# Atomu2014/deep-ctr

Measured on AMD Instinct MI355X. Metric: examples/sec, higher is better.
Workload: dtype bf16; 1 GPU; FNN L3 train step: 16 fields, 937670 one-hot dims, k=10, hidden 300/100 tanh, batch 4096 per GPU, Zipf(1.1) ids; per_gpu_batch=4096, global_batch=4096, parallelism=single

## Files before the change

### deep-ctr_amd/_capi.py

```python
import ctypes as C
import os

_HERE = os.path.dirname(os.path.abspath(__file__))
LIB_PATH = os.environ.get("FNN_HIP_LIB") or os.path.join(_HERE, "libfnn_hip.so")

FNN_OK = 0
FNN_ERR_ARG, FNN_ERR_HIP, FNN_ERR_STATE, FNN_ERR_RANGE, FNN_ERR_NOMEM = -1, -2, -3, -4, -5
FNN_PREC_F32, FNN_PREC_BF16, FNN_PREC_BF16X3 = 0, 1, 2
PRECISIONS = {'f32': FNN_PREC_F32, 'bf16': FNN_PREC_BF16, 'bf16x3': FNN_PREC_BF16X3}
FNN_ACT_TANH, FNN_ACT_SIGMOID, FNN_ACT_LINEAR = 0, 1, 2
FNN_MEM_HOST, FNN_MEM_DEVICE = 0, 1
FNN_MODE_FM, FNN_MODE_BAG = 0, 1
FNN_DP_SPARSE_LOCAL, FNN_DP_SPARSE_EXCHANGE = 0, 1
FNN_DP_PAYLOAD_SLABS, FNN_DP_PAYLOAD_BUCKET = 0, 1
FNN_DP_COLLECTIVE_CALLBACK, FNN_DP_COLLECTIVE_P2P = 0, 1
ALLREDUCE_FN = C.CFUNCTYPE(C.c_int, C.c_void_p, C.c_void_p, C.c_int64, C.c_void_p)
ALLGATHER_FN = C.CFUNCTYPE(C.c_int, C.c_void_p, C.c_void_p, C.c_void_p, C.c_int64, C.c_void_p)


class fnn_cfg(C.Structure):
    _fields_ = [("n_fields", C.c_int32), ("k", C.c_int32), ("hidden1", C.c_int32),
                ("hidden2", C.c_int32), ("max_batch", C.c_int32), ("precision", C.c_int32),
                ("act", C.c_int32), ("reg_all", C.c_int32), ("lr", C.c_float),
                ("lambda1", C.c_float), ("lambda_fm", C.c_float), ("device", C.c_int32),
                ("stream", C.c_void_p), ("mode", C.c_int32), ("h0", C.c_int32)]


_vp, _i, _i64, _f = C.c_void_p, C.c_int, C.c_int64, C.c_float

SIGNATURES = {
    "fnn_version": (C.c_char_p, []),
    "fnn_cfg_size": (C.c_uint64, []),
    "fnn_last_error": (C.c_char_p, [_vp]),
    "fnn_create": (_i, [C.POINTER(fnn_cfg), C.POINTER(_vp)]),
    "fnn_destroy": (_i, [_vp]),
    "fnn_set_hparams": (_i, [_vp, _f, _f, _f]),
    "fnn_stream": (_vp, [_vp]),
    "fnn_sync": (_i, [_vp]),
    "fnn_set_table": (_i, [_vp, _vp, _i64, _vp, _f, _i]),
    "fnn_get_table": (_i, [_vp, _vp, _i]),
    "fnn_get_rows": (_i, [_vp, _vp, _i64, _vp, _i]),
    "fnn_set_dense": (_i, [_vp, _i, _vp, _vp, _i]),
    "fnn_get_dense": (_i, [_vp, _i, _vp, _vp, _i]),
    "fnn_set_bag_bias": (_i, [_vp, _vp, _i]),
    "fnn_get_bag_bias": (_i, [_vp, _vp, _i]),
    "fnn_gather": (_i, [_vp, _vp, _i, _vp, _i]),
    "fnn_train_step": (_i, [_vp, _vp, _vp, _i, _vp, _vp, _i, _vp, _vp, _i, C.POINTER(_f)]),
    "fnn_set_shadowed": (_i, [_vp, _vp, _i, _i]),
# ... 147 lines not shown
```

### deep-ctr_amd/csrc/fm_api.hip

```cpp
#include <hip/hip_runtime.h>

#include <cmath>
#include <cstring>
#include <string>
#include <vector>

#include "../../include/fm_hip.h"
#include "../../include/fnn_hip.h"
#include "fnn_step_kernels.hip.h"
#include "metrics.hip.h"
#include "optim.hip.h"

using namespace fnn;

namespace {

thread_local std::string g_fm_err;
inline int rup(int x, int m) { return (x + m - 1) / m * m; }

struct FmArgs {
    const int32_t* ids; const float* y; int B, F, K; const float* table16; int64_t n_rows; const float* b;
    float scale, dscale; int train; float* gxp; int K1p; float* p_out; float* loss_t; float* gb_part; int* err;
    bool wt;
    int* stamp; int step;
// ... 312 lines not shown
}

}

struct fm_handle {
    std::string err; int dev = 0; hipStream_t st = nullptr; bool own_stream = false;
    int F = 0, K = 0, Bmax = 0, K1p = 0;
    bool wide = false;
    int rw = SLOT;
    int* noshare = nullptr;
    float* table16 = nullptr; int64_t n_rows = 0; float* b = nullptr; double scale = 1.0;
    float *gxp = nullptr, *loss_t = nullptr, *gb_part = nullptr, *loss_dev = nullptr; int* err_flag = nullptr;
    int4* rec = nullptr; double* part = nullptr; int4* owners = nullptr; int* owner_cnt = nullptr; void* skeys = nullptr;
    double* cpow1 = nullptr; bool key64 = true;
    int opt = FM_OPT_SGD; float beta1 = 0.9f, beta2 = 0.999f, eps = 1e-8f; int64_t t = 0; bool dense_g = false;
    int scat_slot = 0;
    int sort_merge4 = 0;
    float *s0 = nullptr, *s1 = nullptr, *sb = nullptr, *G = nullptr; int* stamp = nullptr;
};

#define MHK(h, expr) do { hipError_t e_ = (expr); if (e_ != hipSuccess) { (h)->err = std::string(#expr) + ": " + hipGetErrorString(e_); return FNN_ERR_HIP; } } while (0)
#define MFAIL(h, code, msg) do { (h)->err = (msg); return (code); } while (0)

namespace {

int fold_scale(fm_handle* h)
{
    if (h->scale == 1.0 || !h->table16) return FNN_OK;
    const size_t n = (size_t)h->n_rows * h->rw;
    hipLaunchKernelGGL(k_fm_rescale, dim3((unsigned)((n + 255) / 256)), dim3(256), 0, h->st, h->table16, n, (float)h->scale);
    MHK(h, hipGetLastError());
// ... 127 lines not shown
    }
    {
        SortArgs so{ids, B, F, h->n_rows, h->rec, h->owner_cnt, 4 * F, h->skeys};
        so.merge4 = h->sort_merge4;
        SortArgs sb = so; sb.nblk = 16 * F;
        if (h->key64) {
            hipLaunchKernelGGL((k_sortA<unsigned long long>), dim3(4 * F), dim3(256), sortA_lds_bytes<unsigned long long>(so.merge4), h->st, so);
            launch_fwd<unsigned long long>(h, &sb, a, Ba / 16);
        } else {
            hipLaunchKernelGGL((k_sortA<unsigned>), dim3(4 * F), dim3(256), sortA_lds_bytes<unsigned>(so.merge4), h->st, so);
            launch_fwd<unsigned>(h, &sb, a, Ba / 16);
        }
    }
    if (opt) {
        ScatArgs sa{h->rec, SORT_N, F, h->K, h->gxp, h->K1p, h->cpow1, -1.0, h->G, h->part, h->owner_cnt, h->owners, SLOT};
        const int nsc1 = scat1_blocks(sa, h->scat_slot);
        hipLaunchKernelGGL(k_scat1, dim3(nsc1), dim3(256), 0, h->st, sa);
        hipLaunchKernelGGL(k_fm_scat2_tail, dim3(1 + 256), dim3(256), 0, h->st, sa, h->b, h->gb_part, Ba / 16, lr, lambda, h->loss_t, Ba,
                           reduce_mean ? 1.0f / (float)B : 1.0f, h->loss_dev, FmBiasOpt{h->opt, h->sb, lr_step, h->beta1, h->beta2, h->eps});
        launch_opt_pass(h, lambda, lr_step);
        MHK(h, hipGetLastError());
        return FNN_OK;
    }
    h->scale *= 1.0 - (double)lr * (double)lambda;
    ScatArgs sa{h->rec, SORT_N, F, h->K, h->gxp, h->K1p, h->cpow1, (double)lr / h->scale, h->table16, h->part, h->owner_cnt,
                h->owners, SLOT};
    const int nsc1 = scat1_blocks(sa, h->scat_slot);
    hipLaunchKernelGGL(k_scat1, dim3(nsc1), dim3(256), 0, h->st, sa);
    hipLaunchKernelGGL(k_fm_scat2_tail, dim3(1 + 256), dim3(256), 0, h->st, sa, h->b, h->gb_part, Ba / 16, lr, lambda, h->loss_t, Ba,
                       reduce_mean ? 1.0f / (float)B : 1.0f, h->loss_dev, FmBiasOpt{FM_OPT_SGD, nullptr, 0.f, 0.f, 0.f, 0.f});
    MHK(h, hipGetLastError());
    if (h->scale < 5.96e-8 || h->scale > 1.0) return fold_scale(h);
    return FNN_OK;
}

}

extern "C" {

const char* fm_last_error(const fm_handle* h) { return h ? h->err.c_str() : g_fm_err.c_str(); }

int fm_create(int n_fields, int k, int max_batch, int device, void* stream, fm_handle** out)
// ... 16 lines not shown
    const size_t Ba = rup(h->Bmax, 16);
    FK(al((void**)&h->gxp, Ba * h->K1p * 4)); FK(al((void**)&h->loss_t, Ba * 4)); FK(al((void**)&h->gb_part, (Ba / 8) * 4));
    FK(al((void**)&h->loss_dev, 4)); FK(al((void**)&h->b, 4)); FK(al((void**)&h->err_flag, 4)); FK(al((void**)&h->sb, 8));
    const size_t part_rows = h->wide ? (size_t)h->F * (SORT_N / WCH) * 2 : (size_t)h->F * (SORT_N / 16) * 2;
    FK(al((void**)&h->rec, (size_t)h->F * SORT_N * sizeof(int4))); FK(al((void**)&h->part, part_rows * h->rw * 8));
    FK(al((void**)&h->owners, (size_t)h->F * (SORT_N / 16) * sizeof(int4))); FK(al((void**)&h->owner_cnt, 4));
    FK(al(&h->skeys, (size_t)h->F * SORT_N * 8));
    {
        std::vector<double> ones(SORT_N + 1, 1.0);
        FK(hipMalloc((void**)&h->cpow1, ones.size() * 8));
        FK(hipMemcpy(h->cpow1, ones.data(), ones.size() * 8, hipMemcpyHostToDevice));
    }
    FK(hipStreamSynchronize(h->st));
#undef FK
    h->dense_g = getenv("FM_OPT_DENSE_G") && atoi(getenv("FM_OPT_DENSE_G")) == 1;
    h->scat_slot = scat1_form_env();
    h->sort_merge4 = sort_merge4_env(0);
    *out = h;
    return FNN_OK;
}

int fm_destroy(fm_handle* h)
{
    if (!h) return FNN_ERR_ARG;
    hipSetDevice(h->dev);
    if (h->st) hipStreamSynchronize(h->st);
    void* ptrs[] = {h->table16, h->b, h->gxp, h->loss_t, h->gb_part, h->loss_dev, h->err_flag, h->rec, h->part, h->owners, h->owner_cnt,
                    h->skeys, h->cpow1, h->s0, h->s1, h->sb, h->G, h->stamp, h->noshare};
    for (void* p : ptrs) if (p) hipFree(p);
    if (h->own_stream && h->st) hipStreamDestroy(h->st);
    delete h;
// ... 175 lines not shown
```

### deep-ctr_amd/csrc/fnn_api.hip

```cpp
#include <hip/hip_runtime.h>
#include <rccl/rccl.h>
#include <dlfcn.h>

#include <algorithm>

#include <cmath>
#include <cstdio>
#include <cstdlib>
#include <cstring>
#include <map>
#include <mutex>
#include <string>
#include <vector>

#include "../../include/fnn_hip.h"
#include "fnn_step_kernels.hip.h"
#include "metrics.hip.h"

using namespace fnn;

namespace {

thread_local std::string g_create_err;

// ... 5 lines not shown
}

struct fnn_handle {
    fnn_cfg cfg{};
    std::string err;
    int dev = 0;
    hipStream_t st = nullptr;
    bool own_stream = false;
    int F = 0, K = 0, H1 = 0, H2 = 0, xdim = 0, K1p = 0, H1p = 0, H2p = 0;
    int Bmax = 0, ldT = 0, N2max = 0;
    size_t n1 = 0, n2 = 0, nw12 = 0, nw = 0;
    int splitk = 4;
    int scat2_wgs = 256;
    int sort_merge4 = 1;
    int wgrad_lds = 0;
    int scat_slot = 0;
    bool bf16 = false;
    bool split = false;
    int step1_waves = 8;
    int wt_stores = 47;
    bool bag = false; int rw = SLOT; size_t nbag = 0, off_bag = 0;
    bool wide = false;
    float* bb0 = nullptr; void* dlxT = nullptr; void* onesT = nullptr; float* gx_raw = nullptr;
    bool fused = true;
    int role_off = 0;
    float* table16 = nullptr; int32_t* field_of_row = nullptr; int64_t n_rows = 0; float w0 = 0.f;
    float* master = nullptr; float* bucket = nullptr; float* slab = nullptr;
    void *w1 = nullptr, *w1t = nullptr, *w2 = nullptr, *w2t = nullptr;
    bool dense_set[3] = {false, false, false};
    void *xp = nullptr, *xpT = nullptr, *d1 = nullptr, *d1T = nullptr, *d2 = nullptr, *dl2 = nullptr,
         *dl2T = nullptr, *dl1 = nullptr, *dl1T = nullptr;
// ... 209 lines not shown
}

template <typename T>
void launch_step2(fnn_handle* h, bool dense, bool sparse, const float* gxp_src = nullptr)
{
    const int Ba = h->pend_Ba, nxt = h->cur ^ 1;
    const bool have_next = sparse && h->pend_have_next && !(h->role_off & 1);
    if (h->role_off & 2) dense = false;
    if (h->role_off & 4) sparse = false;
    ScatArgs sa = make_scat_args(h, h->slot[h->cur], SORT_N);
    if (gxp_src) sa.gxp = gxp_src;
    ProfScope ps(h, dense && sparse ? "step2" : (dense ? "step2_dense" : "step2_sparse"), h->st);
    const WgradArgs wa = make_wgrad_args<T>(h, Ba);
    const int nwx = dense ? wgrad_blocks(wa) : 0;
    const int nsc = !sparse ? 0 : (h->bag ? (int)(((size_t)h->F * (SORT_N / WCH) * (h->rw / 4) + 255) / 256)
                                          : scat1_blocks(sa, h->scat_slot));
    SortArgs so{h->next_ids, h->next_B, h->F, h->n_rows, h->slot[nxt].rec, h->slot[nxt].owner_cnt,
                have_next ? 4 * h->F : 0, h->skeys, nullptr, nullptr, 0, h->sort_merge4};
    const dim3 grid(so.nblk + nwx * h->splitk + nsc);
    if (grid.x == 0) return;
    const bool wl = nwx > 0 && h->wgrad_lds && sizeof(T) == 2;
    const size_t lds = std::max(h->key64 ? sortA_lds_bytes<unsigned long long>(so.merge4) : sortA_lds_bytes<unsigned>(so.merge4),
                                wl ? WGRAD_LDS_BYTES : (size_t)0);
#define STEP2(KT, M4, WF) hipLaunchKernelGGL((k_step2<T, KT, M4, WF>), grid, dim3(256), lds, h->st, so, wa, nwx, h->splitk, sa)
#define STEP2_KEYS(WF) do { if (h->key64) { if (so.merge4) STEP2(unsigned long long, true, WF); else STEP2(unsigned long long, false, WF); } \
                            else { if (so.merge4) STEP2(unsigned, true, WF); else STEP2(unsigned, false, WF); } } while (0)
    if constexpr (sizeof(T) == 2) {
        if (wl) { STEP2_KEYS(WGRAD_LDS); return; }
    }
    STEP2_KEYS(WGRAD_DIRECT);
#undef STEP2_KEYS
// ... 289 lines not shown
        sa.gxf = h->rw;
        {
            ProfScope ps(h, "scatter", h->st);
            const size_t nthr = (size_t)F * (N2 / WCH) * (h->rw / 4);
            hipLaunchKernelGGL(k_scatdw1, dim3((unsigned)((nthr + 255) / 256)), dim3(256), 0, h->st, sa);
        }
        {
            ProfScope ps(h, "finalize", h->st);
            hipLaunchKernelGGL(k_scatdw2, dim3(256), dim3(256), 0, h->st, sa);
        }
        HIPCHK(h, hipGetLastError());
        return FNN_OK;
    }
    {
        ProfScope ps(h, "scatter", h->st);
        const int nblk = scat1_blocks(sa, h->scat_slot);
        hipLaunchKernelGGL(k_scat1, dim3(nblk), dim3(256), 0, h->st, sa);
    }
    {
        ProfScope ps(h, "finalize", h->st);
        hipLaunchKernelGGL(k_scat2, dim3(64), dim3(256), 0, h->st, sa);
    }
    HIPCHK(h, hipGetLastError());
    return FNN_OK;
}

int ensure_global_ws(fnn_handle* h, int B_g)
{
    int N2 = sort_n2(B_g);
    if (N2 <= h->gN2 && h->cpow_cap >= B_g + 1) return FNN_OK;
    HIPCHK(h, hipStreamSynchronize(h->st));
// ... 34 lines not shown
            std::string err;
            if (group_global(h->st, ids_g, B_g, F, h->n_rows, N2, sl.rec, sl.owner_cnt, &h->gws, &h->gws_bytes, err) != 0)
                FAIL(h, FNN_ERR_HIP, err);
        } else {
            const int kpt = N2 <= 4096 ? 4 : (N2 == 8192 ? 8 : 16);
            const dim3 blk(N2 / kpt);
            if (kpt == 4) hipLaunchKernelGGL(k_sort<4>, dim3(F), blk, (size_t)N2 * 8, h->st, ids_g, B_g, F, h->n_rows, N2, sl.rec, sl.owner_cnt, nullptr, 0, h->err_flag);
            else if (kpt == 8) hipLaunchKernelGGL(k_sort<8>, dim3(F), blk, (size_t)N2 * 8, h->st, ids_g, B_g, F, h->n_rows, N2, sl.rec, sl.owner_cnt, nullptr, 0, h->err_flag);
            else hipLaunchKernelGGL(k_sort<16>, dim3(F), blk, (size_t)N2 * 8, h->st, ids_g, B_g, F, h->n_rows, N2, sl.rec, sl.owner_cnt, nullptr, 0, h->err_flag);
        }
    }
    {
        ProfScope ps(h, "scatter_global", h->st);
        ScatArgs sa = make_scat_args(h, sl, N2);
        sa.gxp = gxp_g;
        const int nblk = scat1_blocks(sa, h->scat_slot);
        hipLaunchKernelGGL(k_scat1, dim3(nblk), dim3(256), 0, h->st, sa);
        hipLaunchKernelGGL(k_scat2, dim3(N2 > 4096 ? 256 : 64), dim3(256), 0, h->st, sa);
    }
    HIPCHK(h, hipGetLastError());
    h->next_ids = nullptr; h->next_B = 0;
    h->scatter_pending = false;
    return FNN_OK;
}

struct RcclApi {
    void* lib = nullptr;
    decltype(&ncclGetUniqueId) GetUniqueId = nullptr;
    decltype(&ncclCommInitRank) CommInitRank = nullptr;
    decltype(&ncclAllReduce) AllReduce = nullptr;
    decltype(&ncclAllGather) AllGather = nullptr;
// ... 81 lines not shown
    if (!h->table16) FAIL(h, FNN_ERR_STATE, "fnn_set_table has not been called");
    if (!(h->dense_set[0] && h->dense_set[1] && h->dense_set[2]))
        FAIL(h, FNN_ERR_STATE, "fnn_set_dense has not been called for all three layers");
    return FNN_OK;
}

}

extern "C" {

const char* fnn_version(void) { return "fnn_hip 0.2 (gfx950)"; }

uint64_t fnn_cfg_size(void) { return (uint64_t)sizeof(fnn_cfg); }

const char* fnn_last_error(const fnn_handle* h) { return h ? h->err.c_str() : g_create_err.c_str(); }

int fnn_create(const fnn_cfg* cfg, fnn_handle** out)
{
    if (!cfg || !out) { g_create_err = "null argument"; return FNN_ERR_ARG; }
    *out = nullptr;
    if (cfg->n_fields < 2 || cfg->n_fields > 64) { g_create_err = "n_fields must be in [2, 64]"; return FNN_ERR_ARG; }
    if (cfg->mode != FNN_MODE_FM && cfg->mode != FNN_MODE_BAG) { g_create_err = "bad mode"; return FNN_ERR_ARG; }
    if (cfg->mode == FNN_MODE_BAG && (cfg->h0 < 192 || cfg->h0 > 316 || cfg->h0 % 4 != 0)) {
        g_create_err = "FNN_MODE_BAG: h0 must be a multiple of 4 in [192, 316] (the strip kernel is built for bag rows of 256 or 320 padded floats; the reference uses 200 and 300, python/SNN_RBM.py:25,53)"; return FNN_ERR_ARG; }
    if (cfg->mode == FNN_MODE_FM && (cfg->k < 1 || cfg->k > 128 || cfg->k == 16)) {
        g_create_err = "k = rank+1 must be in [1, 15] (two pad slots of the 16-float row carry w_0 and the bias) or in [17, 128] (wide rows of rup(k, 4) floats); k = 16 is not supported"; return FNN_ERR_ARG; }
    if (cfg->mode == FNN_MODE_FM && cfg->k >= 17 && cfg->n_fields * rup(cfg->k, 4) > WIDE_XW_MAX) {
        g_create_err = "k >= 17: n_fields * rup(k, 4) must be <= 4096 (the layer-one width of the wide-row path)"; return FNN_ERR_ARG; }
    if (cfg->hidden1 < 1 || cfg->hidden1 > 4095 || cfg->hidden2 < 1 || cfg->hidden2 > 255) { g_create_err = "hidden1 must be in [1, 4095], hidden2 in [1, 255]"; return FNN_ERR_ARG; }
    if (cfg->max_batch < 1 || cfg->max_batch > 16384) { g_create_err = "max_batch must be in [1, 16384] (per-field LDS sort)"; return FNN_ERR_ARG; }
// ... 20 lines not shown
    h->xdim = 1 + h->F * h->K;
    h->K1p = rup(h->F * SLOT, 64); h->H1p = rup(h->H1 + 1, 64); h->H2p = rup(h->H2 + 1, 64);
    h->bag = cfg->mode == FNN_MODE_BAG;
    if (const char* e = getenv("FNN_WT_STORES")) h->wt_stores = atoi(e);
    if (const char* e = getenv("FNN_STEP1_WAVES")) h->step1_waves = atoi(e) == 4 ? 4 : 8;
    if (h->bag) { h->rw = cfg->h0; h->K = cfg->h0; h->xdim = cfg->h0; h->K1p = rup(cfg->h0 + 1, 64); }
    h->wide = !h->bag && h->K >= 17;
    if (h->wide) { h->rw = rup(h->K, 4); h->K1p = rup(h->F * h->rw + 2, 64); }
    h->Bmax = cfg->max_batch; h->ldT = rup(h->Bmax, 256);
    h->N2max = SORT_N; while (h->N2max < h->Bmax) h->N2max <<= 1;
    h->n1 = (size_t)h->K1p * h->H1p; h->n2 = (size_t)h->H1p * h->H2p;
    h->nw12 = h->n1 + h->n2; h->nw = h->nw12 + h->H2p;
    h->bf16 = cfg->precision == FNN_PREC_BF16; h->split = cfg->precision == FNN_PREC_BF16X3;
    if (const char* ev = getenv("FNN_NO_FUSE")) h->fused = !(ev[0] == '1');
    if (const char* ev = getenv("FNN_ROLE_OFF")) h->role_off = atoi(ev);
    h->scat_slot = scat1_form_env();
    h->sort_merge4 = sort_merge4_env(h->bag ? 0 : 1);
    const bool steps3 = h->fused && mlp_shape_ok(h) && !h->bag && !h->scat_slot && !h->split && h->Bmax <= SORT_N;
    if (steps3) h->splitk = 8;
    const bool lds_dflt = steps3 && h->bf16 && h->ldT / 4 / Traits<bf16_t>::KS >= WGRAD_LDS_S;
    h->wgrad_lds = wgrad_form == WGRAD_LDS || (wgrad_form == -1 && lds_dflt) ? 1 : 0;
    if (wgrad_form == -1 && lds_dflt) h->splitk = 4;
    if (const char* ev = getenv("FNN_SPLITK")) { const int v = atoi(ev); if (v == 2 || v == 4 || v == 8 || v == 16) h->splitk = v; }
    if (const char* ev = getenv("FNN_SCAT2_WGS")) { const int v = atoi(ev); if (v >= 16 && v <= 1024) h->scat2_wgs = v; }
    const size_t ts = tsize(h), Ba = h->ldT;
    CK(alloc_dev(h, &h->master, h->nw));
    h->off_bag = h->nw12 + (size_t)h->H2p * 64;
    h->nbag = h->bag ? (size_t)h->K1p : 0;
    CK(alloc_dev(h, &h->bucket, h->nw + h->nbag));
    h->nslab = h->off_bag + h->nbag * 64;
    CK(alloc_dev(h, &h->slab, (size_t)h->splitk * h->nslab));
    CK(alloc_dev(h, (char**)&h->w1, h->n1 * ts));   CK(alloc_dev(h, (char**)&h->w1t, h->n1 * ts));
    CK(alloc_dev(h, (char**)&h->w2, h->n2 * ts));   CK(alloc_dev(h, (char**)&h->w2t, h->n2 * ts));
// ... 763 lines not shown
```

### deep-ctr_amd/csrc/fnn_kernels.hip.h

```cpp
#pragma once
#include <hip/hip_runtime.h>
#include <stdint.h>
#include <stdlib.h>
#include <string.h>
#include <type_traits>

namespace fnn {

typedef __bf16 bf16_t;
typedef __bf16 bf16x8 __attribute__((ext_vector_type(8)));
typedef __bf16 bf16x4 __attribute__((ext_vector_type(4)));
typedef float f32x4 __attribute__((ext_vector_type(4)));

constexpr int SLOT = 16;
constexpr int ACT_TANH = 0, ACT_SIGMOID = 1, ACT_LINEAR = 2;
constexpr double FIX_SCALE = 17592186044416.0;

__host__ __device__ inline unsigned bs_pack(const float v) {
    const bf16_t h = (bf16_t)v;
    const bf16_t l = (bf16_t)(v - (float)h);
    return (unsigned)__builtin_bit_cast(unsigned short, h) | (unsigned)__builtin_bit_cast(unsigned short, l) << 16;
}
__host__ __device__ inline float bs_unpack(const unsigned u) {
    return __builtin_bit_cast(float, u << 16) + __builtin_bit_cast(float, u & 0xffff0000u);
// ... 1619 lines not shown
            const int s = lo;
            lo = pos + 1; hi = N2;
            while (lo < hi) { const int mid = (lo + hi) >> 1; if (s_key[mid] < hi_key) lo = mid + 1; else hi = mid; }
            r = make_int4((int)(kk >> 32), (int)(kk & 0xffffffffu), s, lo);
        }
        rec[(size_t)f * N2 + pos] = r;
    }
}

struct ScatArgs {
    const int4* rec; int N2, F, K; const float* gxp; int K1p; const double* cpow; double lr;
    float* table16; double* part; int* owner_cnt; int4* owners;
    int rw;
    const int* tag_shared; int stamp;
    int gxf;
    int slot_form;
};
__device__ __forceinline__ void atomic_add4(float* p, float a, float b, float c, float d) {
    atomicAdd(p, a); atomicAdd(p + 1, b); atomicAdd(p + 2, c); atomicAdd(p + 3, d);
}
__device__ __forceinline__ void scat1_body(const ScatArgs& sa, const int blk)
{
    const int4* __restrict__ rec = sa.rec; const int N2 = sa.N2, F = sa.F, K = sa.K, K1p = sa.K1p;
    const float* __restrict__ gxp = sa.gxp; const double* __restrict__ cpow = sa.cpow; const double lr = sa.lr;
    float* __restrict__ table16 = sa.table16; double* __restrict__ part = sa.part;
    int* __restrict__ owner_cnt = sa.owner_cnt; int4* __restrict__ owners = sa.owners;
    const int l = threadIdx.x & 15;
    const int G = (blk * 256 + threadIdx.x) >> 4;
    const int NQ = N2 >> 4;
    if (G >= F * NQ) return;
    const int f = G / NQ, q = G % NQ, base = q * 16;
    const int4 mine = rec[(size_t)f * N2 + base + l];
// ... 89 lines not shown
                    if (lim < 3) o.z = wold[j].z;
                    o.w = wold[j].w;
                }
                *reinterpret_cast<float4*>(sa.table16 + (size_t)r[j].x * SLOT + 4 * q) = o;
            } else {
                const int which = (s < base) ? 0 : 1;
                double* pp = sa.part + (((size_t)f * NQ + qc) * 2 + which) * SLOT + 4 * q;
                pp[0] = a0; pp[1] = a1; pp[2] = a2; pp[3] = a3;
                if (which == 1 && q == 0) sa.owners[atomicAdd(sa.owner_cnt, 1)] = make_int4(f, s, e, r[j].x);
            }
            a0 = a1 = a2 = a3 = 0;
        }
    }
}

static __global__ __launch_bounds__(256) void k_scat1(const ScatArgs sa)
{
    if (sa.slot_form) scat1_body(sa, blockIdx.x);
    else scat1q_body(sa, blockIdx.x);
}

inline int scat1_blocks(ScatArgs& sa, const int slot_form)
{
    const bool vec_ok = ((uintptr_t)sa.gxp | (uintptr_t)sa.table16) % 16 == 0 && sa.K1p % 4 == 0;
    sa.slot_form = (slot_form || !vec_ok) ? 1 : 0;
    const size_t nthr = sa.slot_form ? (size_t)sa.F * sa.N2 : (size_t)sa.F * (sa.N2 / 16) * ((sa.K + 3) / 4);
    return (int)((nthr + 255) / 256);
}
inline int scat1_form_env()
{
    const char* e = getenv("FNN_SCAT1_FORM");
    return e && !strcmp(e, "slot") ? 1 : 0;
}

__device__ __forceinline__ void scat2_body(const ScatArgs& sa, const int blk, const int nblk, double (*s_sum)[16])
{
    const int4* __restrict__ owners = sa.owners; const int N2 = sa.N2, K = sa.K;
    const double* __restrict__ part = sa.part; const double* __restrict__ cpow = sa.cpow; const double lr = sa.lr;
    float* __restrict__ table16 = sa.table16;
    const int n = *sa.owner_cnt;
    const int l = threadIdx.x & 15, grp = threadIdx.x >> 4;
    const int NQ = N2 >> 4;
    for (int o = blk; o < n; o += nblk) {
        const int4 ow = owners[o];
        const int q0 = ow.y >> 4, q1 = (ow.z - 1) >> 4;
        double sum = 0.0;
        float* p = table16 + (size_t)ow.w * SLOT + l;
// ... 311 lines not shown
```

### deep-ctr_amd/csrc/fnn_step_kernels.hip.h

```cpp
#pragma once
#include "fnn_kernels.hip.h"

namespace fnn {

template <typename KT> struct KeyTraits;
template <> struct KeyTraits<unsigned> { static constexpr int SH = 12; };
template <> struct KeyTraits<unsigned long long> { static constexpr int SH = 32; };

struct SortArgs {
    const int32_t* ids; int B, F; int64_t n_rows; int4* rec; int* owner_cnt; int nblk; void* skeys;
    int* tag_first; int* tag_shared; int stamp;
    int merge4;
};

constexpr int SORT_N = 4096;

template <typename KT> __host__ __device__ constexpr size_t sort_lds_bytes() { return (size_t)SORT_N * sizeof(KT); }
template <typename KT> inline size_t sortA_lds_bytes(const int merge4) { return merge4 ? (size_t)1024 * sizeof(KT) : 0; }
inline int sort_merge4_env(const int dflt)
{
    const char* e = getenv("FNN_SORT_RUNS");
    const int v = e ? atoi(e) : 0;
    return v == 16 ? 0 : (v == 4 ? 1 : dflt);
}
// ... 191 lines not shown
static __global__ __launch_bounds__(256) void k_step2(const SortArgs so, const WgradArgs wa, const int nwx,
                                               const int splitk, const ScatArgs sa)
{
    extern __shared__ __align__(16) unsigned char smem[];
    const int b = blockIdx.x, nw = nwx * splitk;
    if (b < so.nblk) sortA_form<KT, M4>(so, b, smem);
    else if (b < so.nblk + nw) {
        int w = b - so.nblk;
        if (((b ^ w) & 7) == 0) {
            const int cls = w & 7, k = w >> 3, qd = nw >> 3, rm = nw & 7;
            w = (cls < rm ? cls * (qd + 1) : rm * (qd + 1) + (cls - rm) * qd) + k;
        }
        wgrad_body<T, WF>(wa, w % nwx, w / nwx, smem);
    }
    else if (sa.rw != SLOT) scatw1_body(sa, b - so.nblk - nw);
    else if (sa.slot_form) scat1_body(sa, b - so.nblk - nw);
    else scat1q_body(sa, b - so.nblk - nw);
}

struct TailArgs {
    const float* slab; int splitk; size_t nw_all, nw12, nslab; float* master; float lambda1; int reg_all;
    const float* loss_t; int Ba; float* bucket; float* loss_sum; float lr; int K1p, H1p, H2p;
    void *w1, *w1t, *w2, *w2t; int nblk_red;
    float* bb0; size_t nbag, off_bag;
};

template <typename T, bool UPDATE, typename KT, bool M4>
static __global__ __launch_bounds__(256) void k_step3(const SortArgs so, const TailArgs ta, const ScatArgs sa)
{
    extern __shared__ __align__(16) unsigned char smem[];
    __shared__ double s_sum[16][16];
// ... 148 lines not shown
```

### deep-ctr_amd/csrc/ipnn_api.hip

```cpp
#include <hip/hip_runtime.h>

#include <algorithm>
#include <cmath>
#include <cstring>
#include <map>
#include <string>
#include <vector>

#include "../../include/fnn_hip.h"
#include "../../include/ipnn_hip.h"
#include "fnn_step_kernels.hip.h"
#include "metrics.hip.h"
#include "optim.hip.h"

using namespace fnn;

namespace {

thread_local std::string g_ip_err;
inline int rup(int x, int m) { return (x + m - 1) / m * m; }

constexpr int A_TANH = IPNN_ACT_TANH, A_SIG = IPNN_ACT_SIGMOID, A_RELU = IPNN_ACT_RELU;

__device__ inline float ip_act(float z, int act) {
// ... 1337 lines not shown
    bool upd_side = false, tab_pending = false, upd_pending = false;
    float* emb = nullptr;
    float *dz0 = nullptr, *gxp = nullptr, *gb_part = nullptr, *loss_t = nullptr, *loss_dev = nullptr, *slab = nullptr;
    int* ref0 = nullptr; int* err_flag = nullptr;
    int4* rec = nullptr; double* part = nullptr; int4* owners = nullptr; int* owner_cnt = nullptr; void* skeys = nullptr;
    double* cpow1 = nullptr; bool key64 = true;
    size_t slab_stride = 0;
    bool prof = false;
    long long* stamps = nullptr;
    bool group_wgrad = true;
    bool strip_attr = false;
    int mask_side = 0;
    int group_xcd = 1;
    int strip_rot = 1, fwd_skip = 0;
    int wide_nf = 2, wide_nw = 8;
    int scat_slot = 0;
    int sort_merge4 = 1;
    bool wt = true;
    int tail_fuse = 1;
    int tail_nf = 1;
    int tail_nw = 16;
    int ipf_nt = 1024;
    int strip_warm = 1;
    bool strip = true;
    int duo = 1, duo_min = DUO_MIN_BLOCKS;
    unsigned long long* duo_xch = nullptr; int* duo_flags = nullptr; int duo_epoch = 0; size_t duo_xch_wg = 0; int n_cu = 256;
    bool stamp_tail = false;
    int tail_split = 1;
    bool duo_failed = false;
    bool gemm_lds = false;
    std::map<std::string, std::vector<std::pair<hipEvent_t, hipEvent_t>>> prof_ev;
// ... 395 lines not shown
            }
            hipLaunchKernelGGL(k_ip_b_update, dim3(1), dim3(256), 0, ss, h->b, h->gb_part, ngb, h->adam ? (int)h->cfg.optimizer : 0, h->bmv,
                               lr_step, h->cfg.adam_beta1, h->cfg.adam_beta2, h->cfg.adam_eps, h->err_flag);
        }
        if (h->wide) {
            IpProf ps(h, "scatter", ss);
            ScatArgs sa{h->rec, SORT_N, F, h->K, h->gxp, h->Dp[0], h->cpow1, h->adam ? -1.0 : (double)h->cfg.lr,
                        h->adam ? h->tG : h->table16, h->part, h->owner_cnt, h->owners, h->rw, h->noshare, 1, h->rw};
            const int nthr = F * (SORT_N / WCH) * (h->rw / 4);
            hipLaunchKernelGGL(k_ip_scatw1, dim3((nthr + 255) / 256), dim3(256), 0, ss, sa);
            hipLaunchKernelGGL(k_ip_scatw2, dim3(256), dim3(256), 0, ss, sa);
        } else {
            IpProf ps(h, "scatter", ss);
            ScatArgs sa{h->rec, SORT_N, F, h->K, h->gxp, h->Dp[0], h->cpow1, h->adam ? -1.0 : (double)h->cfg.lr,
                        h->adam ? h->tG : h->table16, h->part, h->owner_cnt, h->owners, SLOT};
            const int nsc1 = scat1_blocks(sa, h->scat_slot);
            hipLaunchKernelGGL(k_scat1, dim3(nsc1), dim3(256), 0, ss, sa);
            hipLaunchKernelGGL(k_scat2, dim3(256), dim3(256), 0, ss, sa);
        }
        if (h->adam) {
            IpProf ps(h, "adam_table", ss);
            const size_t n = (size_t)h->n_rows * h->rw;
            hipLaunchKernelGGL(k_adam_table, dim3((unsigned)((n / 4 + 255) / 256)), dim3(256), 0, ss, h->table16, h->tm, h->tv, h->tG, n,
                               lr_step, h->cfg.adam_beta1, h->cfg.adam_beta2, h->cfg.adam_eps, (int)h->cfg.optimizer);
        }
        if (h->st2) IHK(h, hipEventRecord(h->st2 && h->upd_side ? h->ev_tab : h->ev_join, h->st2));
    }
    {
        IpProf ps(h, "wgrad");
        if (h->group_wgrad && L + 1 <= GEMM_GROUP_MAX) {
            GemmGroupArgs g{};
// ... 80 lines not shown
    h->wide = h->K > SLOT; h->rw = h->wide ? rup(h->K, 4) : SLOT;
    h->P = cfg->pairs ? h->F * (h->F - 1) / 2 : 0; h->CB = h->F * h->rw + h->P; h->bf16 = cfg->precision == FNN_PREC_BF16;
    h->Bmax = cfg->max_batch; h->ldT = rup(h->Bmax, 256);
    if (const char* e = getenv("IPNN_GEMM_LDS")) h->gemm_lds = atoi(e) != 0;
    if (const char* e = getenv("IPNN_STRIP")) h->strip = atoi(e) != 0;
    if (const char* e = getenv("IPNN_STRIP_DUO")) h->duo = atoi(e);
    if (const char* e = getenv("IPNN_DUO_MIN")) h->duo_min = std::max(2, atoi(e));
    if (const char* e = getenv("IPNN_TAIL_SPLIT")) h->tail_split = atoi(e);
    { int ncu = 0; if (hipDeviceGetAttribute(&ncu, hipDeviceAttributeMultiprocessorCount, cfg->device) == hipSuccess && ncu > 0) h->n_cu = ncu; }
    if (const char* e = getenv("IPNN_STRIP_ROT")) h->strip_rot = atoi(e);
    if (const char* e = getenv("IPNN_STRIP_WARM")) h->strip_warm = atoi(e);
    if (const char* e = getenv("IPNN_UPDATE_SIDE")) h->upd_side = atoi(e) != 0;
    if (const char* e = getenv("IPNN_IPF_NT")) h->ipf_nt = atoi(e) == 1024 ? 1024 : 512;
    if (const char* e = getenv("IPNN_TAIL_FUSE")) h->tail_fuse = atoi(e) != 0;
    if (const char* e = getenv("IPNN_WT")) h->wt = atoi(e) != 0;
    h->scat_slot = scat1_form_env();
    h->sort_merge4 = sort_merge4_env(1);
    if (const char* e = getenv("IPNN_WIDE")) { int nf = 4, nw = 8; if (sscanf(e, "%d:%d", &nf, &nw) == 2 && ((nf == 2 && (nw == 8 || nw == 12)) || (nf == 4 && nw == 8))) { h->wide_nf = nf; h->wide_nw = nw; } }
    if (const char* e = getenv("IPNN_TAIL_NW")) h->tail_nw = atoi(e) == 16 ? 16 : 8;
    if (const char* e = getenv("IPNN_TAIL_NF")) { const int v = atoi(e); if (v == 1 || v == 2 || v == 4) h->tail_nf = v; }
    if (const char* e = getenv("IPNN_GROUP_XCD")) h->group_xcd = atoi(e);
    if (const char* e = getenv("IPNN_MASK_SIDE")) h->mask_side = atoi(e);
    if (const char* e = getenv("IPNN_FWD_SKIP")) h->fwd_skip = atoi(e);
    const char* side = getenv("IPNN_SIDE_STREAM");
    if (const char* e = getenv("IPNN_GROUP_WGRAD")) h->group_wgrad = atoi(e) != 0;
    auto fail = [&](int code) { g_ip_err = h->err; ipnn_destroy(h); return code; };
#define IK(expr) do { hipError_t e2_ = (expr); if (e2_ != hipSuccess) { h->err = std::string(#expr) + ": " + hipGetErrorString(e2_); return fail(FNN_ERR_HIP); } } while (0)
    IK(hipSetDevice(h->dev));
    if (cfg->stream) h->st = (hipStream_t)cfg->stream; else { IK(hipStreamCreateWithFlags(&h->st, hipStreamNonBlocking)); h->own_stream = true; }
    if (!side || atoi(side) != 0) {
        IK(hipStreamCreateWithFlags(&h->st2, hipStreamNonBlocking));
// ... 408 lines not shown
```

### include/fnn_hip.h

```cpp
#ifndef FNN_HIP_H
#define FNN_HIP_H

#include <stdint.h>

#ifdef __cplusplus
extern "C" {
#endif
#if defined(__GNUC__)
#pragma GCC visibility push(default)
#endif

#define FNN_OK          0
#define FNN_ERR_ARG    -1
#define FNN_ERR_HIP    -2
#define FNN_ERR_STATE  -3
#define FNN_ERR_RANGE  -4
#define FNN_ERR_NOMEM  -5

#define FNN_PREC_F32    0
#define FNN_PREC_BF16   1
#define FNN_PREC_BF16X3 2

#define FNN_ACT_TANH    0
#define FNN_ACT_SIGMOID 1
// ... 16 lines not shown
    int32_t reg_all;
    float   lr;
    float   lambda1;
    float   lambda_fm;
    int32_t device;
    void*   stream;
    int32_t mode;
    int32_t h0;
} fnn_cfg;

typedef struct fnn_handle fnn_handle;

const char* fnn_version(void);
uint64_t fnn_cfg_size(void);
const char* fnn_last_error(const fnn_handle* h);

int fnn_create(const fnn_cfg* cfg, fnn_handle** out);
int fnn_destroy(fnn_handle* h);
int fnn_set_hparams(fnn_handle* h, float lr, float lambda1, float lambda_fm);
void* fnn_stream(fnn_handle* h);
int fnn_sync(fnn_handle* h);

int fnn_set_table(fnn_handle* h, const float* rows, int64_t n_rows,
                  const int32_t* field_of_row, float w0, int memkind);
int fnn_get_table(fnn_handle* h, float* rows_out, int memkind);
int fnn_get_rows(fnn_handle* h, const int64_t* row_ids, int64_t n, float* out, int memkind);

int fnn_set_dense(fnn_handle* h, int layer, const float* W, const float* b, int memkind);
int fnn_get_dense(fnn_handle* h, int layer, float* W, float* b, int memkind);

// ... 61 lines not shown
```

Baseline: 122.1 million examples/sec.

## Add half-chunk scatter kernel form with DPP carry and make it default

Adds a new scatter-1 variant in which two lanes share each 16-row sorted chunk, eight rows each. The lower half's running segment sum is passed to the upper lane through a DPP lane shift, and this form becomes the default over the quarter form. The aim is to double thread-level parallelism and shorten each thread's serial chain of loads and accumulations in the sparse embedding update. In exchange, gxp and cpow loads are duplicated per half, and correctness now depends on the adjacent-lane DPP pattern.

```diff
diff --git a/deep-ctr_amd/_capi.py b/deep-ctr_amd/_capi.py
--- a/deep-ctr_amd/_capi.py
+++ b/deep-ctr_amd/_capi.py
@@ -32,6 +32,7 @@
     "fnn_version": (C.c_char_p, []),
     "fnn_cfg_size": (C.c_uint64, []),
     "fnn_last_error": (C.c_char_p, [_vp]),
+    "fnn_scat1_form": (C.c_char_p, []),
     "fnn_create": (_i, [C.POINTER(fnn_cfg), C.POINTER(_vp)]),
     "fnn_destroy": (_i, [_vp]),
     "fnn_set_hparams": (_i, [_vp, _f, _f, _f]),
diff --git a/deep-ctr_amd/csrc/fm_api.hip b/deep-ctr_amd/csrc/fm_api.hip
--- a/deep-ctr_amd/csrc/fm_api.hip
+++ b/deep-ctr_amd/csrc/fm_api.hip
@@ -350,7 +350,7 @@
     int4* rec = nullptr; double* part = nullptr; int4* owners = nullptr; int* owner_cnt = nullptr; void* skeys = nullptr;
     double* cpow1 = nullptr; bool key64 = true;
     int opt = FM_OPT_SGD; float beta1 = 0.9f, beta2 = 0.999f, eps = 1e-8f; int64_t t = 0; bool dense_g = false;
-    int scat_slot = 0;
+    int scat_form = SCAT1_HALF;
     int sort_merge4 = 0;
     float *s0 = nullptr, *s1 = nullptr, *sb = nullptr, *G = nullptr; int* stamp = nullptr;
 };
@@ -508,7 +508,7 @@
     }
     if (opt) {
         ScatArgs sa{h->rec, SORT_N, F, h->K, h->gxp, h->K1p, h->cpow1, -1.0, h->G, h->part, h->owner_cnt, h->owners, SLOT};
-        const int nsc1 = scat1_blocks(sa, h->scat_slot);
+        const int nsc1 = scat1_blocks(sa, h->scat_form);
         hipLaunchKernelGGL(k_scat1, dim3(nsc1), dim3(256), 0, h->st, sa);
         hipLaunchKernelGGL(k_fm_scat2_tail, dim3(1 + 256), dim3(256), 0, h->st, sa, h->b, h->gb_part, Ba / 16, lr, lambda, h->loss_t, Ba,
                            reduce_mean ? 1.0f / (float)B : 1.0f, h->loss_dev, FmBiasOpt{h->opt, h->sb, lr_step, h->beta1, h->beta2, h->eps});
@@ -519,7 +519,7 @@
     h->scale *= 1.0 - (double)lr * (double)lambda;
     ScatArgs sa{h->rec, SORT_N, F, h->K, h->gxp, h->K1p, h->cpow1, (double)lr / h->scale, h->table16, h->part, h->owner_cnt,
                 h->owners, SLOT};
-    const int nsc1 = scat1_blocks(sa, h->scat_slot);
+    const int nsc1 = scat1_blocks(sa, h->scat_form);
     hipLaunchKernelGGL(k_scat1, dim3(nsc1), dim3(256), 0, h->st, sa);
     hipLaunchKernelGGL(k_fm_scat2_tail, dim3(1 + 256), dim3(256), 0, h->st, sa, h->b, h->gb_part, Ba / 16, lr, lambda, h->loss_t, Ba,
                        reduce_mean ? 1.0f / (float)B : 1.0f, h->loss_dev, FmBiasOpt{FM_OPT_SGD, nullptr, 0.f, 0.f, 0.f, 0.f});
@@ -566,7 +566,7 @@
     FK(hipStreamSynchronize(h->st));
 #undef FK
     h->dense_g = getenv("FM_OPT_DENSE_G") && atoi(getenv("FM_OPT_DENSE_G")) == 1;
-    h->scat_slot = scat1_form_env();
+    h->scat_form = scat1_form_env();
     h->sort_merge4 = sort_merge4_env(0);
     *out = h;
     return FNN_OK;
diff --git a/deep-ctr_amd/csrc/fnn_api.hip b/deep-ctr_amd/csrc/fnn_api.hip
--- a/deep-ctr_amd/csrc/fnn_api.hip
+++ b/deep-ctr_amd/csrc/fnn_api.hip
@@ -43,7 +43,7 @@
     int scat2_wgs = 256;
     int sort_merge4 = 1;
     int wgrad_lds = 0;
-    int scat_slot = 0;
+    int scat_form = SCAT1_HALF;
     bool bf16 = false;
     bool split = false;
     int step1_waves = 8;
@@ -283,7 +283,7 @@
     const WgradArgs wa = make_wgrad_args<T>(h, Ba);
     const int nwx = dense ? wgrad_blocks(wa) : 0;
     const int nsc = !sparse ? 0 : (h->bag ? (int)(((size_t)h->F * (SORT_N / WCH) * (h->rw / 4) + 255) / 256)
-                                          : scat1_blocks(sa, h->scat_slot));
+                                          : scat1_blocks(sa, h->scat_form));
     SortArgs so{h->next_ids, h->next_B, h->F, h->n_rows, h->slot[nxt].rec, h->slot[nxt].owner_cnt,
                 have_next ? 4 * h->F : 0, h->skeys, nullptr, nullptr, 0, h->sort_merge4};
     const dim3 grid(so.nblk + nwx * h->splitk + nsc);
@@ -603,7 +603,7 @@
     }
     {
         ProfScope ps(h, "scatter", h->st);
-        const int nblk = scat1_blocks(sa, h->scat_slot);
+        const int nblk = scat1_blocks(sa, h->scat_form);
         hipLaunchKernelGGL(k_scat1, dim3(nblk), dim3(256), 0, h->st, sa);
     }
     {
@@ -668,7 +668,7 @@
         ProfScope ps(h, "scatter_global", h->st);
         ScatArgs sa = make_scat_args(h, sl, N2);
         sa.gxp = gxp_g;
-        const int nblk = scat1_blocks(sa, h->scat_slot);
+        const int nblk = scat1_blocks(sa, h->scat_form);
         hipLaunchKernelGGL(k_scat1, dim3(nblk), dim3(256), 0, h->st, sa);
         hipLaunchKernelGGL(k_scat2, dim3(N2 > 4096 ? 256 : 64), dim3(256), 0, h->st, sa);
     }
@@ -780,6 +780,12 @@
 uint64_t fnn_cfg_size(void) { return (uint64_t)sizeof(fnn_cfg); }
 
 const char* fnn_last_error(const fnn_handle* h) { return h ? h->err.c_str() : g_create_err.c_str(); }
+
+const char* fnn_scat1_form(void)
+{
+    const int f = scat1_form_env(-1);
+    return f == SCAT1_SLOT ? "slot" : f == SCAT1_QUARTER ? "quarter" : f == SCAT1_HALF ? "half" : "default";
+}
 
 int fnn_create(const fnn_cfg* cfg, fnn_handle** out)
 {
@@ -830,9 +836,9 @@
     h->bf16 = cfg->precision == FNN_PREC_BF16; h->split = cfg->precision == FNN_PREC_BF16X3;
     if (const char* ev = getenv("FNN_NO_FUSE")) h->fused = !(ev[0] == '1');
     if (const char* ev = getenv("FNN_ROLE_OFF")) h->role_off = atoi(ev);
-    h->scat_slot = scat1_form_env();
+    h->scat_form = scat1_form_env();
     h->sort_merge4 = sort_merge4_env(h->bag ? 0 : 1);
-    const bool steps3 = h->fused && mlp_shape_ok(h) && !h->bag && !h->scat_slot && !h->split && h->Bmax <= SORT_N;
+    const bool steps3 = h->fused && mlp_shape_ok(h) && !h->bag && h->scat_form != SCAT1_SLOT && !h->split && h->Bmax <= SORT_N;
     if (steps3) h->splitk = 8;
     const bool lds_dflt = steps3 && h->bf16 && h->ldT / 4 / Traits<bf16_t>::KS >= WGRAD_LDS_S;
     h->wgrad_lds = wgrad_form == WGRAD_LDS || (wgrad_form == -1 && lds_dflt) ? 1 : 0;
diff --git a/deep-ctr_amd/csrc/fnn_kernels.hip.h b/deep-ctr_amd/csrc/fnn_kernels.hip.h
--- a/deep-ctr_amd/csrc/fnn_kernels.hip.h
+++ b/deep-ctr_amd/csrc/fnn_kernels.hip.h
@@ -1657,8 +1657,9 @@
     int rw;
     const int* tag_shared; int stamp;
     int gxf;
-    int slot_form;
+    int form;
 };
+enum { SCAT1_QUARTER = 0, SCAT1_SLOT = 1, SCAT1_HALF = 2 };
 __device__ __forceinline__ void atomic_add4(float* p, float a, float b, float c, float d) {
     atomicAdd(p, a); atomicAdd(p + 1, b); atomicAdd(p + 2, c); atomicAdd(p + 3, d);
 }
@@ -1778,23 +1779,100 @@
     }
 }
 
+__device__ __forceinline__ double lane_below(const double v)
+{
+    const int lo = __builtin_amdgcn_update_dpp(0, __double2loint(v), 0xA0, 0xf, 0xf, false);
+    const int hi = __builtin_amdgcn_update_dpp(0, __double2hiint(v), 0xA0, 0xf, 0xf, false);
+    return __hiloint2double(hi, lo);
+}
+
+__device__ __forceinline__ void scat1h_body(const ScatArgs& sa, const int blk)
+{
+    const int N2 = sa.N2, NQ = N2 >> 4, nq = (sa.K + 3) >> 2;
+    const int gid = blk * 256 + (int)threadIdx.x;
+    const int half = gid & 1, cq = gid >> 1;
+    const int chunk = cq / nq, q = cq % nq;
+    if (chunk >= sa.F * NQ) return;
+    const int f = chunk / NQ, qc = chunk % NQ, base = qc * 16, hb = base + 8 * half;
+    const int lim = sa.K - 4 * q;
+    const double* __restrict__ cpow = sa.cpow; const double lr = sa.lr;
+    int4 r[8];
+#pragma unroll
+    for (int j = 0; j < 8; ++j) r[j] = sa.rec[(size_t)f * N2 + hb + j];
+    float4 g[8], wold[8];
+    double wd[8], cs[8];
+#pragma unroll
+    for (int j = 0; j < 8; ++j) {
+        const int pos = hb + j;
+        const bool live = r[j].x >= 0;
+        g[j] = *reinterpret_cast<const float4*>(sa.gxp + (size_t)(live ? r[j].y : 0) * sa.K1p + f * SLOT + 4 * q);
+        const bool need = live && pos + 1 == r[j].w && r[j].z >= base;
+        wold[j] = *reinterpret_cast<const float4*>(sa.table16 + (size_t)(need ? r[j].x : 0) * SLOT + 4 * q);
+        wd[j] = cpow[live ? r[j].w - 1 - pos : 0];
+        cs[j] = cpow[need ? r[j].w - r[j].z : 0];
+    }
+    if (lim < 4) {
+#pragma unroll
+        for (int j = 0; j < 8; ++j) {
+            if (lim < 2) g[j].y = 0.f;
+            if (lim < 3) g[j].z = 0.f;
+            g[j].w = 0.f;
+        }
+    }
+    double a0 = 0, a1 = 0, a2 = 0, a3 = 0;
+#pragma unroll
+    for (int j = 0; j < 8; ++j) {
+        if (r[j].x < 0) continue;
+        a0 += (double)g[j].x * wd[j]; a1 += (double)g[j].y * wd[j]; a2 += (double)g[j].z * wd[j]; a3 += (double)g[j].w * wd[j];
+        if (hb + j + 1 == r[j].w) a0 = a1 = a2 = a3 = 0;
+    }
+    a0 = lane_below(a0); a1 = lane_below(a1); a2 = lane_below(a2); a3 = lane_below(a3);
+    if (!half) a0 = a1 = a2 = a3 = 0;
+#pragma unroll
+    for (int j = 0; j < 8; ++j) {
+        if (r[j].x < 0) continue;
+        a0 += (double)g[j].x * wd[j]; a1 += (double)g[j].y * wd[j]; a2 += (double)g[j].z * wd[j]; a3 += (double)g[j].w * wd[j];
+        const int pos = hb + j, s = r[j].z, e = r[j].w;
+        if (pos + 1 != e && pos + 1 != base + 16) continue;
+        if (s >= base && e <= base + 16) {
+            float4 o = make_float4((float)((double)wold[j].x * cs[j] - lr * a0), (float)((double)wold[j].y * cs[j] - lr * a1),
+                                   (float)((double)wold[j].z * cs[j] - lr * a2), (float)((double)wold[j].w * cs[j] - lr * a3));
+            if (lim < 4) {
+                if (lim < 2) o.y = wold[j].y;
+                if (lim < 3) o.z = wold[j].z;
+                o.w = wold[j].w;
+            }
+            *reinterpret_cast<float4*>(sa.table16 + (size_t)r[j].x * SLOT + 4 * q) = o;
+        } else {
+            const int which = (s < base) ? 0 : 1;
+            double* pp = sa.part + (((size_t)f * NQ + qc) * 2 + which) * SLOT + 4 * q;
+            pp[0] = a0; pp[1] = a1; pp[2] = a2; pp[3] = a3;
+            if (which == 1 && q == 0) sa.owners[atomicAdd(sa.owner_cnt, 1)] = make_int4(f, s, e, r[j].x);
+        }
+        a0 = a1 = a2 = a3 = 0;
+    }
+}
+
 static __global__ __launch_bounds__(256) void k_scat1(const ScatArgs sa)
 {
-    if (sa.slot_form) scat1_body(sa, blockIdx.x);
+    if (sa.form == SCAT1_SLOT) scat1_body(sa, blockIdx.x);
+    else if (sa.form == SCAT1_HALF) scat1h_body(sa, blockIdx.x);
     else scat1q_body(sa, blockIdx.x);
 }
 
-inline int scat1_blocks(ScatArgs& sa, const int slot_form)
+inline int scat1_blocks(ScatArgs& sa, const int form)
 {
     const bool vec_ok = ((uintptr_t)sa.gxp | (uintptr_t)sa.table16) % 16 == 0 && sa.K1p % 4 == 0;
-    sa.slot_form = (slot_form || !vec_ok) ? 1 : 0;
-    const size_t nthr = sa.slot_form ? (size_t)sa.F * sa.N2 : (size_t)sa.F * (sa.N2 / 16) * ((sa.K + 3) / 4);
+    sa.form = vec_ok ? form : SCAT1_SLOT;
+    const size_t nquarters = (size_t)sa.F * (sa.N2 / 16) * ((sa.K + 3) / 4);
+    const size_t nthr = sa.form == SCAT1_SLOT ? (size_t)sa.F * sa.N2 : sa.form == SCAT1_HALF ? 2 * nquarters : nquarters;
     return (int)((nthr + 255) / 256);
 }
-inline int scat1_form_env()
+inline int scat1_form_env(const int dflt = SCAT1_HALF)
 {
     const char* e = getenv("FNN_SCAT1_FORM");
-    return e && !strcmp(e, "slot") ? 1 : 0;
+    if (!e) return dflt;
+    return !strcmp(e, "slot") ? SCAT1_SLOT : !strcmp(e, "quarter") ? SCAT1_QUARTER : !strcmp(e, "half") ? SCAT1_HALF : dflt;
 }
 
 __device__ __forceinline__ void scat2_body(const ScatArgs& sa, const int blk, const int nblk, double (*s_sum)[16])
diff --git a/deep-ctr_amd/csrc/fnn_step_kernels.hip.h b/deep-ctr_amd/csrc/fnn_step_kernels.hip.h
--- a/deep-ctr_amd/csrc/fnn_step_kernels.hip.h
+++ b/deep-ctr_amd/csrc/fnn_step_kernels.hip.h
@@ -229,7 +229,8 @@
         wgrad_body<T, WF>(wa, w % nwx, w / nwx, smem);
     }
     else if (sa.rw != SLOT) scatw1_body(sa, b - so.nblk - nw);
-    else if (sa.slot_form) scat1_body(sa, b - so.nblk - nw);
+    else if (sa.form == SCAT1_SLOT) scat1_body(sa, b - so.nblk - nw);
+    else if (sa.form == SCAT1_HALF) scat1h_body(sa, b - so.nblk - nw);
     else scat1q_body(sa, b - so.nblk - nw);
 }
 
diff --git a/deep-ctr_amd/csrc/ipnn_api.hip b/deep-ctr_amd/csrc/ipnn_api.hip
--- a/deep-ctr_amd/csrc/ipnn_api.hip
+++ b/deep-ctr_amd/csrc/ipnn_api.hip
@@ -1375,7 +1375,7 @@
     int group_xcd = 1;
     int strip_rot = 1, fwd_skip = 0;
     int wide_nf = 2, wide_nw = 8;
-    int scat_slot = 0;
+    int scat_form = SCAT1_HALF;
     int sort_merge4 = 1;
     bool wt = true;
     int tail_fuse = 1;
@@ -1801,7 +1801,7 @@
             IpProf ps(h, "scatter", ss);
             ScatArgs sa{h->rec, SORT_N, F, h->K, h->gxp, h->Dp[0], h->cpow1, h->adam ? -1.0 : (double)h->cfg.lr,
                         h->adam ? h->tG : h->table16, h->part, h->owner_cnt, h->owners, SLOT};
-            const int nsc1 = scat1_blocks(sa, h->scat_slot);
+            const int nsc1 = scat1_blocks(sa, h->scat_form);
             hipLaunchKernelGGL(k_scat1, dim3(nsc1), dim3(256), 0, ss, sa);
             hipLaunchKernelGGL(k_scat2, dim3(256), dim3(256), 0, ss, sa);
         }
@@ -1912,7 +1912,7 @@
     if (const char* e = getenv("IPNN_IPF_NT")) h->ipf_nt = atoi(e) == 1024 ? 1024 : 512;
     if (const char* e = getenv("IPNN_TAIL_FUSE")) h->tail_fuse = atoi(e) != 0;
     if (const char* e = getenv("IPNN_WT")) h->wt = atoi(e) != 0;
-    h->scat_slot = scat1_form_env();
+    h->scat_form = scat1_form_env();
     h->sort_merge4 = sort_merge4_env(1);
     if (const char* e = getenv("IPNN_WIDE")) { int nf = 4, nw = 8; if (sscanf(e, "%d:%d", &nf, &nw) == 2 && ((nf == 2 && (nw == 8 || nw == 12)) || (nf == 4 && nw == 8))) { h->wide_nf = nf; h->wide_nw = nw; } }
     if (const char* e = getenv("IPNN_TAIL_NW")) h->tail_nw = atoi(e) == 16 ? 16 : 8;
diff --git a/include/fnn_hip.h b/include/fnn_hip.h
--- a/include/fnn_hip.h
+++ b/include/fnn_hip.h
@@ -54,6 +54,7 @@
 const char* fnn_version(void);
 uint64_t fnn_cfg_size(void);
 const char* fnn_last_error(const fnn_handle* h);
+const char* fnn_scat1_form(void);
 
 int fnn_create(const fnn_cfg* cfg, fnn_handle** out);
 int fnn_destroy(fnn_handle* h);
```

After: 132.2 million examples/sec, median of 6. 1.08x the previous value.
